# yaoyx689/RigGS

Hardware: AMD Instinct MI355X
Metric: train iters/sec (deform+raster fwd+bwd), 300k Gaussians @800x800 (higher is better)
Workload: dtype f32; 1 GPU; 300k Gaussians / 24-joint skeleton / 800x800, LBS-only, SH degree 3, anisotropic, one frame per GPU per step; num_gaussians=300000, num_joints=24, tile_instances_R=1963607, tile_lists=canonical: upstream's ceil(3 sigma) squares (the library default), parallelism=frames x1, launch=hipGraph replay

## Files before the change

### riggs_amd/csrc/pose_mlp.hip

```cpp
#include "fk_device.h"

namespace riggs {

#define PM_MAX_LAYERS 12
#define PM_MAX_W 256
#define PM_MAX_HEAD 320
#define PM_MAX_IN 320
#define PM_MAX_EMB 64
#define PM_RPW 8
#define PM_NG 16
#define PM_CPL 5

struct PoseMlpDesc {
  int depth;
  int width;
  int multires;
  int skip;
  int n_rot;
  const float* W[PM_MAX_LAYERS];
  const float* b[PM_MAX_LAYERS];
  const float *W_rot, *b_rot, *W_tr, *b_tr;
};

__device__ __forceinline__ int pm_in_dim(const PoseMlpDesc& d, int l, int emb) {
  if (l == 0) return emb;
  return (l - 1 == d.skip) ? d.width + emb : d.width;
}


__device__ __forceinline__ float pm_input(const PoseMlpDesc& d, const float* __restrict__ acts, int l, int emb, int i) {
  if (l == 0) return acts[i];
  if (l - 1 == d.skip) return (i < emb) ? acts[i] : acts[emb + (size_t)(l - 1) * d.width + (i - emb)];
  return acts[emb + (size_t)(l - 1) * d.width + i];
}

__global__ __launch_bounds__(64) void pm_embed_kernel(PoseMlpDesc d, const float* __restrict__ t, float* __restrict__ acts) {
  const int tid = threadIdx.x, emb = 1 + 2 * d.multires;
  if (tid < emb) {
    const float tv = t[0];
    float v = tv;
    if (tid > 0) {
      const int k = (tid - 1) >> 1;
      const float f = (float)(1 << k);
      v = ((tid - 1) & 1) ? cosf(tv * f) : sinf(tv * f);
    }
    acts[tid] = v;
  }
}

__global__ __launch_bounds__(256) void pm_layer_kernel(PoseMlpDesc d, int l, float* __restrict__ acts,
                                                       const float* __restrict__ rot_bias4,
                                                       float* __restrict__ rotation, float* __restrict__ translation) {
  const int lane = threadIdx.x & 63, wave = threadIdx.x >> 6;
  const int emb = 1 + 2 * d.multires;
  const bool heads = (l == d.depth);
  const int n_out = heads ? d.n_rot + 3 : d.width;
  const int r = blockIdx.x * 4 + wave;
  if (r >= n_out) return;
  const int in_dim = pm_in_dim(d, l, emb);
  const float* row;
  float bias;
  if (!heads) { row = d.W[l] + (size_t)r * in_dim; bias = d.b[l][r]; }
  else if (r < d.n_rot) { row = d.W_rot + (size_t)r * in_dim; bias = d.b_rot[r]; }
  else { row = d.W_tr + (size_t)(r - d.n_rot) * in_dim; bias = d.b_tr[r - d.n_rot]; }
  float acc = 0.f;
#pragma unroll
  for (int k = 0; k < PM_CPL; k++) {
    const int i = lane + 64 * k;
    if (i < in_dim) acc += row[i] * pm_input(d, acts, l, emb, i);
  }
  acc = wave_sum(acc);
  if (lane == 63) {
    const float v = acc + bias;
    if (!heads) acts[emb + (size_t)l * d.width + r] = fmaxf(v, 0.f);
    else if (r < d.n_rot) rotation[r] = rot_bias4 ? v + rot_bias4[r & 3] : v;
    else translation[r - d.n_rot] = v;
  }
}

#define PM_RG 8
__global__ __launch_bounds__(256) void pm_backward_step_kernel(PoseMlpDesc d, int l, const float* __restrict__ acts,
                                                               const float* __restrict__ g_rot,
                                                               const float* __restrict__ g_tr,
                                                               const float* __restrict__ dh_out ,
                                                               float* __restrict__ dh_in , float* __restrict__ dzs) {
  __shared__ float s_part[4][64];
  const int tid = threadIdx.x, lane = tid & 63, wave = tid >> 6;
  const int emb = 1 + 2 * d.multires;
  const bool heads = (l == d.depth);
  const int n_rows = heads ? d.n_rot + 3 : d.width;
  const int in_dim = pm_in_dim(d, l, emb);
  const int off = (l == d.skip) ? emb : 0;
  const int c = blockIdx.x * 64 + lane;
  const int rstep = 4 * PM_RG, r0 = blockIdx.y * 4 + wave;
  float acc = 0.f;
#pragma unroll 4
  for (int r = r0; r < n_rows; r += rstep) {
    float v;
    const float* row;
    if (heads) {
      v = (r < d.n_rot) ? g_rot[r] : g_tr[r - d.n_rot];
      row = (r < d.n_rot) ? d.W_rot + (size_t)r * in_dim : d.W_tr + (size_t)(r - d.n_rot) * in_dim;
    } else {
      const float h = acts[emb + (size_t)l * d.width + r];
      v = (h > 0.f) ? dh_out[off + r] : 0.f;
      row = d.W[l] + (size_t)r * in_dim;
      if (blockIdx.x == 0 && lane == 0) dzs[(size_t)l * d.width + r] = v;
    }
    if (l > 0 && c < in_dim) acc += row[c] * v;
  }
  if (l == 0) return;
  s_part[wave][lane] = acc;
  __syncthreads();
  if (wave == 0 && c < in_dim) atomicAdd(&dh_in[c], s_part[0][lane] + s_part[1][lane] + s_part[2][lane] + s_part[3][lane]);
}

struct PoseMlpGradDesc {
  int64_t w_off[PM_MAX_LAYERS + 2];
  int64_t b_off[PM_MAX_LAYERS + 2];
  int row_start[PM_MAX_LAYERS + 3];
};
__global__ __launch_bounds__(64) void pm_backward_weights_kernel(PoseMlpDesc d, PoseMlpGradDesc g,
                                                                 const float* __restrict__ acts,
                                                                 const float* __restrict__ dzs,
                                                                 const float* __restrict__ g_rot,
                                                                 const float* __restrict__ g_tr,
                                                                 float* __restrict__ flat) {
  const int emb = 1 + 2 * d.multires;
  const int nmat = d.depth + 2;
  int m = 0;
  while (m + 1 < nmat && (int)blockIdx.x >= g.row_start[m + 1]) m++;
  const int r = blockIdx.x - g.row_start[m];
  const int l = (m < d.depth) ? m : d.depth;
  const int in_dim = pm_in_dim(d, l, emb);
  const float v = (m < d.depth) ? dzs[(size_t)m * d.width + r] : (m == d.depth ? g_rot[r] : g_tr[r]);
  float* out = flat + g.w_off[m] + (size_t)r * in_dim;
  for (int c = threadIdx.x; c < in_dim; c += 64) out[c] = v * pm_input(d, acts, l, emb, c);
  if (threadIdx.x == 0) flat[g.b_off[m] + r] = v;
}


#define PMF_WAVES 8
#define PM_TRACE(i) do { if (trace && blockIdx.x == 0 && threadIdx.x == 0) trace[i] = wall_clock64(); } while (0)
#define PMF_SPIN_MAX (1u << 17)
typedef __attribute__((address_space(1))) unsigned long long pm_gu64;

__device__ __forceinline__ void pm_store_granule(unsigned long long* g, uint32_t tag, float value, bool local) {
  const unsigned long long x = ((unsigned long long)tag << 32) | (unsigned long long)__float_as_uint(value);
  if (local) asm volatile("global_store_dwordx2 %0, %1, off" ::"v"(g), "v"(x) : "memory");
  else __hip_atomic_store((pm_gu64*)g, x, __ATOMIC_RELAXED, __HIP_MEMORY_SCOPE_AGENT);
}

__device__ __forceinline__ void pm_sweep_issue(pm_gu64* g, int n, int lane, unsigned long long (&x)[4]) {
#pragma unroll
  for (int k = 0; k < 4; k++) {
    const int r = lane + 64 * k;
    x[k] = (r < n) ? __hip_atomic_load(g + r, __ATOMIC_RELAXED, __HIP_MEMORY_SCOPE_AGENT) : 0ull;
  }
}
__device__ __forceinline__ bool pm_sweep_check(const unsigned long long (&x)[4], int n, int lane, uint32_t tag,
                                               float (&v)[4]) {
  bool ok = true;
#pragma unroll
  for (int k = 0; k < 4; k++) {
    v[k] = __uint_as_float((uint32_t)x[k]);
    if (lane + 64 * k < n) ok &= ((uint32_t)(x[k] >> 32) == tag);
  }
  return __all(ok);
}
template <int NQ>
__device__ __forceinline__ bool pm_sweep_n(const unsigned long long* gran, int n, uint32_t tag, float (&v)[4],
                                           uint32_t* err, uint32_t* sticky, int lane) {
  pm_gu64* g = (pm_gu64*)gran;
  unsigned long long x[NQ][4];
#pragma unroll
  for (int q = 0; q < NQ; q++) {
    pm_sweep_issue(g, n, lane, x[q]);
    __builtin_amdgcn_s_sleep(2);
  }
  for (uint32_t spins = 0;; spins++) {
#pragma unroll
    for (int q = 0; q < NQ; q++) {
      if (pm_sweep_check(x[q], n, lane, tag, v)) return true;
      pm_sweep_issue(g, n, lane, x[q]);
    }
    if (spins > PMF_SPIN_MAX / NQ) {
      if (lane == 0) { atomicOr(err, 1u); if (sticky) atomicOr(sticky, 1u); }
      return false;
    }
  }
}
__device__ __forceinline__ bool pm_sweep(const unsigned long long* gran, int n, uint32_t tag, float (&v)[4],
                                         uint32_t* err, uint32_t* sticky, int lane, bool local = false) {
  return local ? pm_sweep_n<2>(gran, n, tag, v, err, sticky, lane) : pm_sweep_n<4>(gran, n, tag, v, err, sticky, lane);
}

#define PM_CHAIN_STRIDE 8
#define PM_MAX_CHAIN 64
__device__ __forceinline__ bool pm_chain_is_local(unsigned long long* xg, int rank, int n_chain, uint32_t tag, uint32_t* err,
                                                  uint32_t* sticky, int lane, int wave, int* s_word, int by = 0) {
  if (wave == by) {
    const uint32_t mine = __builtin_amdgcn_s_getreg(63508) & 0xFu;
    if (lane == 0) pm_store_granule(xg + rank, tag, __uint_as_float(mine), false);
    float v[4];
    const bool ok = pm_sweep(xg, n_chain, tag, v, err, sticky, lane);
    const bool same = ok && (lane >= n_chain || __float_as_uint(v[0]) == mine);
    const bool all_same = __all(same);
    if (lane == 0) *s_word = all_same ? 1 : 0;
  }
  __syncthreads();
  return *s_word != 0;
}

#define PM_FAULT_BIT 1u
__global__ __launch_bounds__(PMF_WAVES * 64) void pm_forward_fused_kernel(PoseMlpDesc d, const float* __restrict__ t,
                                                                          const float* __restrict__ rot_bias4,
                                                                          float* __restrict__ acts,
                                                                          unsigned long long* gran, uint32_t* gen,
                                                                          uint32_t* sticky, uint32_t* bwd_state, int bwd_words,
                                                                          float* __restrict__ rotation,
                                                                          float* __restrict__ translation,
                                                                          float* __restrict__ wt, int n_chain, int stride,
                                                                          unsigned long long* xcc_gran,
                                                                          unsigned long long* trace) {
  __shared__ float s_in[PM_MAX_IN];
  __shared__ int s_failed, s_local;
  const int lane = threadIdx.x & 63, wave = threadIdx.x >> 6;
  const int rank = (int)blockIdx.x / stride;
  if ((int)blockIdx.x % stride != 0 || rank >= n_chain) {
    __shared__ float s_t[32][33];
    const int emb_ = 1 + 2 * d.multires;
    const int tx = threadIdx.x & 31, ty = threadIdx.x >> 5;
    const int tiles_per = (PM_MAX_HEAD / 32) * (PM_MAX_W / 32);
    const int n_side = (int)gridDim.x - n_chain, side = (int)blockIdx.x - min(n_chain, (int)blockIdx.x / stride + 1);
    for (int tile = side; tile < d.depth * tiles_per; tile += n_side) {
      const int l = 1 + tile / tiles_per, tt = tile % tiles_per;
      const int r0 = (tt / (PM_MAX_W / 32)) * 32, c0 = (tt % (PM_MAX_W / 32)) * 32;
      const bool heads = (l == d.depth);
      const int in_dim = pm_in_dim(d, l, emb_);
      const int off = (l - 1 == d.skip) ? emb_ : 0;
      const int n_rows = heads ? d.n_rot + 3 : d.width;
#pragma unroll
      for (int h = 0; h < 2; h++) {
        const int r = r0 + ty + 16 * h, c = c0 + tx;
        float v = 0.f;
        if (r < n_rows && c < d.width) {
          const float* rp = !heads ? d.W[l] + (size_t)r * in_dim
                                   : (r < d.n_rot ? d.W_rot + (size_t)r * in_dim : d.W_tr + (size_t)(r - d.n_rot) * in_dim);
          v = rp[off + c];
        }
        s_t[ty + 16 * h][tx] = v;
      }
      __syncthreads();
#pragma unroll
      for (int h = 0; h < 2; h++)
        wt[((size_t)(l - 1) * PM_MAX_W + c0 + ty + 16 * h) * PM_MAX_HEAD + r0 + tx] = s_t[tx][ty + 16 * h];
      __syncthreads();
    }
    return;
  }
  const int row = rank * PMF_WAVES + wave;
  const int emb = 1 + 2 * d.multires;
  uint32_t* err = bwd_state;
  for (int i = rank * blockDim.x + threadIdx.x; i < bwd_words; i += n_chain * blockDim.x) bwd_state[i] = 0u;
  const uint32_t tag0 = __hip_atomic_load((__attribute__((address_space(1))) uint32_t*)gen, __ATOMIC_RELAXED,
                                          __HIP_MEMORY_SCOPE_AGENT) * 32u;
  float w[PM_MAX_LAYERS + 1][PM_CPL];
  float bias[PM_MAX_LAYERS + 1];
#pragma unroll
  for (int l = 0; l <= PM_MAX_LAYERS; l++) {
    bias[l] = 0.f;
#pragma unroll
    for (int k = 0; k < PM_CPL; k++) w[l][k] = 0.f;
    if (l <= d.depth) {
      const bool heads = (l == d.depth);
      const int n_out = heads ? d.n_rot + 3 : d.width;
      const int in_dim = pm_in_dim(d, l, emb);
      if (row < n_out) {
        const float* rp;
        if (!heads) { rp = d.W[l] + (size_t)row * in_dim; bias[l] = d.b[l][row]; }
        else if (row < d.n_rot) { rp = d.W_rot + (size_t)row * in_dim; bias[l] = d.b_rot[row]; }
        else { rp = d.W_tr + (size_t)(row - d.n_rot) * in_dim; bias[l] = d.b_tr[row - d.n_rot]; }
#pragma unroll
        for (int k = 0; k < PM_CPL; k++) {
          const int i = lane + 64 * k;
          if (i < in_dim) w[l][k] = rp[i];
        }
      }
    }
  }
  float embv = 0.f;
  if (lane < emb) {
    const float tv = t[0];
    embv = tv;
    if (lane > 0) {
      const int kf = (lane - 1) >> 1;
      const float f = (float)(1 << kf);
      embv = ((lane - 1) & 1) ? cosf(tv * f) : sinf(tv * f);
    }
    if (wave == 0) s_in[lane] = embv;
    if (wave == 0 && rank == 0) acts[lane] = embv;
  }
  if (threadIdx.x == 0) s_failed = 0;
  const bool fault = sticky != nullptr && rank == 1 && (sticky[1] & PM_FAULT_BIT) != 0u;
  PM_TRACE(0);
  const bool local = pm_chain_is_local(xcc_gran, rank, n_chain, tag0 + 31u, err, sticky, lane, wave, &s_local);
  const bool extra = rank * PMF_WAVES >= d.width;
#pragma unroll
  for (int l = 0; l <= PM_MAX_LAYERS; l++) {
    if (l <= d.depth && !(extra && l < d.depth)) {
      const bool heads = (l == d.depth);
      const int n_out = heads ? d.n_rot + 3 : d.width;
      const int in_dim = pm_in_dim(d, l, emb);
      PM_TRACE(1 + 2 * l);
      if (l > 0) {
        if (wave == 0) {
          float v[4];
          bool ok = (s_failed == 0);
          if (ok) ok = pm_sweep(gran + (size_t)(l - 1) * d.width, d.width, tag0 + (uint32_t)l, v, err, sticky, lane, local);
          if (!ok && lane == 0) s_failed = 1;
          const int off = (l - 1 == d.skip) ? emb : 0;
          if (off > 0 && lane < emb) s_in[lane] = embv;
#pragma unroll
          for (int k = 0; k < 4; k++) {
            const int r = lane + 64 * k;
            if (r < d.width) s_in[off + r] = v[k];
          }
        }
        __syncthreads();
      }
      float acc = 0.f;
#pragma unroll
      for (int k = 0; k < PM_CPL; k++) {
        const int i = lane + 64 * k;
        if (i < in_dim) acc += w[l][k] * s_in[i];
      }
      acc = wave_sum(acc);
      PM_TRACE(2 + 2 * l);
      if (lane == 63 && row < n_out) {
        float v = acc + bias[l];
        if (s_failed) v = __builtin_nanf("");
        if (!heads) {
          v = s_failed ? v : fmaxf(v, 0.f);
          if (!(fault && l == 1)) pm_store_granule(gran + (size_t)l * d.width + row, tag0 + (uint32_t)(l + 1), v, local);
          acts[emb + (size_t)l * d.width + row] = v;
        } else if (row < d.n_rot) {
          rotation[row] = rot_bias4 ? v + rot_bias4[row & 3] : v;
        } else {
          translation[row - d.n_rot] = v;
        }
      }
      __syncthreads();
    }
  }
  if (rank == 0 && threadIdx.x == 0)
    __hip_atomic_store((__attribute__((address_space(1))) uint32_t*)gen, tag0 / 32u + 1u, __ATOMIC_RELAXED,
                       __HIP_MEMORY_SCOPE_AGENT);
}

struct PmFkArgs {
  int J;
  const float *local_rot, *joints;
  const int32_t* parents;
  const float *dG, *g_nodes;
  const float* transforms;
  float *dq_out, *dgt_out;
  const float* fixed_coef;
  float* fixed_loss_out;
};

__global__ __launch_bounds__(256) void pm_fixed_add_kernel(int J, const float* __restrict__ local_rot, const float* __restrict__ coef,
                                                           float* __restrict__ dq, float* __restrict__ loss_out) {
  __shared__ float s_p[4];
  float ss = 0.f;
  for (int t = threadIdx.x; t < 4 * J; t += 256) {
    const float d = local_rot[t] - ((t & 3) == 0 ? 1.f : 0.f);
    if (coef) dq[t] += coef[0] * d;
    ss += d * d;
  }
  for (int o = 32; o > 0; o >>= 1) ss += __shfl_xor(ss, o);
  if ((threadIdx.x & 63) == 0) s_p[threadIdx.x >> 6] = ss;
  __syncthreads();
  if (threadIdx.x == 0 && loss_out) loss_out[0] = ((s_p[0] + s_p[1]) + (s_p[2] + s_p[3])) / (float)(4 * J);
}
__global__ __launch_bounds__(256) void pm_add_kernel(int n, const float* __restrict__ src, float* __restrict__ dst) {
  const int i = blockIdx.x * 256 + threadIdx.x;
  if (i < n) dst[i] += src[i];
}

#undef PM_FAULT_BIT
#define PM_FAULT_BIT 2u
__global__ __launch_bounds__(PMF_WAVES * 64) void pm_backward_fused_kernel(PoseMlpDesc d, PoseMlpGradDesc g, PmFkArgs fk,
                                                                           const float* __restrict__ acts,
                                                                           const float* __restrict__ g_rot,
                                                                           const float* __restrict__ g_tr,
                                                                           unsigned long long* gran, uint32_t* err,
                                                                           uint32_t* sticky, uint32_t* gen, float* __restrict__ flat,
                                                                           const float* __restrict__ wt, int n_chain, int stride,
                                                                           unsigned long long* xcc_gran,
                                                                           unsigned long long* trace) {
  __shared__ float s_v[PM_MAX_HEAD];
  __shared__ int s_failed, s_local;
  const int lane = threadIdx.x & 63, wave = threadIdx.x >> 6;
  const int rank = (int)blockIdx.x / stride;
  if ((int)blockIdx.x % stride != 0 || rank >= n_chain) return;
  const int col = rank * PMF_WAVES + wave;
  const bool extra = rank * PMF_WAVES >= d.width;
  const int emb = 1 + 2 * d.multires;
  const int n_head = d.n_rot + 3;
  const uint32_t tag0 = __hip_atomic_load((__attribute__((address_space(1))) uint32_t*)gen, __ATOMIC_RELAXED,
                                          __HIP_MEMORY_SCOPE_AGENT) * 32u;
  __shared__ float s_gq[4 * MAX_J + 4];
  FkIn fin;
  if (fk.J > 0 && wave == 0) fk_load(fk.J, fk.local_rot, fk.joints, fk.parents, fk.dG, fk.g_nodes, fin, fk.transforms);
  float wc[PM_MAX_LAYERS + 1][4];
  float wc_head = 0.f;
#pragma unroll
  for (int l = 1; l <= PM_MAX_LAYERS; l++) {
#pragma unroll
    for (int k = 0; k < 4; k++) wc[l][k] = 0.f;
    if (l <= d.depth && col < d.width) {
      const int n_rows = (l == d.depth) ? n_head : d.width;
      const float* rp = wt + ((size_t)(l - 1) * PM_MAX_W + col) * PM_MAX_HEAD;
#pragma unroll
      for (int k = 0; k < 4; k++) {
        const int r = lane + 64 * k;
        if (r < n_rows) wc[l][k] = rp[r];
      }
      if (l == d.depth && lane + 256 < n_rows) wc_head = rp[lane + 256];
    }
  }
  __shared__ float s_acts[PM_MAX_EMB + PM_MAX_LAYERS * PM_MAX_W];
  __shared__ float s_late[PM_MAX_LAYERS + 1];
  for (int i = threadIdx.x; i < emb + d.depth * d.width; i += blockDim.x) s_acts[i] = acts[i];
  if (threadIdx.x == 0) s_failed = 0;
  const bool fault = sticky != nullptr && rank == 1 && (sticky[1] & PM_FAULT_BIT) != 0u;
  PM_TRACE(0);
  if (fk.J > 0 && wave == 0) {
    FkLane f;
    fk_wave_forward(fk.J, fin, f, fk.transforms != nullptr);
    float dq[4];
    fk_wave_backward(fk.J, fin, f, dq);
    if (lane < fk.J) {
#pragma unroll
      for (int e = 0; e < 4; e++) s_gq[4 * lane + e] = dq[e];
    }
  }
  const bool local = pm_chain_is_local(xcc_gran, rank, n_chain, tag0 + 31u, err, sticky, lane, wave, &s_local, 1);
  if (fk.J > 0) {
    if (threadIdx.x < 3) {
      float sgt = g_tr ? g_tr[threadIdx.x] : 0.f;
      if (fk.g_nodes) for (int k = 0; k < fk.J; k++) sgt += fk.g_nodes[3 * k + threadIdx.x];
      s_gq[4 * fk.J + threadIdx.x] = sgt;
      if (rank == 0 && fk.dgt_out) fk.dgt_out[threadIdx.x] = sgt;
    }
    __syncthreads();
    if (g_rot && (int)threadIdx.x < 4 * fk.J) s_gq[threadIdx.x] += g_rot[threadIdx.x];
    if ((fk.fixed_coef || fk.fixed_loss_out) && wave == 0) {
      float ss = 0.f;
      for (int i = lane; i < 4 * fk.J; i += 64) {
        const float dqf = fk.local_rot[i] - ((i & 3) == 0 ? 1.f : 0.f);
        ss += dqf * dqf;
      }
      for (int o = 32; o > 0; o >>= 1) ss += __shfl_xor(ss, o);
      if (rank == 0 && lane == 0 && fk.fixed_loss_out) fk.fixed_loss_out[0] = ss / (float)(4 * fk.J);
    }
    if (fk.fixed_coef && (int)threadIdx.x < 4 * fk.J)
      s_gq[threadIdx.x] += fk.fixed_coef[0] * (fk.local_rot[threadIdx.x] - ((threadIdx.x & 3) == 0 ? 1.f : 0.f));
    __syncthreads();
    if (rank == 0 && fk.dq_out && (int)threadIdx.x < 4 * fk.J) fk.dq_out[threadIdx.x] = s_gq[threadIdx.x];
  }
  PM_TRACE(1);
#pragma unroll
  for (int l = PM_MAX_LAYERS; l >= 0; l--) {
    if (l <= d.depth && !(extra && l < d.depth)) {
      const bool heads = (l == d.depth);
      const int n_rows = heads ? n_head : d.width;
      const int in_dim = pm_in_dim(d, l, emb);
      PM_TRACE(2 + 2 * (d.depth - l));
      if (wave == 0) {
        if (heads) {
#pragma unroll
          for (int k = 0; k < PM_MAX_HEAD / 64; k++) {
            const int r = lane + 64 * k;
            if (fk.J > 0) s_v[r] = (r < n_head) ? s_gq[r] : 0.f;
            else s_v[r] = (r < d.n_rot) ? g_rot[r] : (r < n_head ? g_tr[r - d.n_rot] : 0.f);
          }
        } else {
          float h[4];
#pragma unroll
          for (int k = 0; k < 4; k++) {
            const int r = lane + 64 * k;
            h[k] = (r < d.width) ? s_acts[emb + (size_t)l * d.width + r] : 0.f;
          }
          float v[4];
          bool ok = (s_failed == 0);
          if (ok) ok = pm_sweep(gran + (size_t)l * d.width, d.width, tag0 + (uint32_t)(l + 1), v, err, sticky, lane, local);
          if (!ok && lane == 0) s_failed = 1;
#pragma unroll
          for (int k = 0; k < 4; k++) {
            const int r = lane + 64 * k;
            if (r < PM_MAX_W) s_v[r] = (r < d.width && h[k] > 0.f) ? v[k] : 0.f;
          }
        }
      }
      __syncthreads();
      PM_TRACE(3 + 2 * (d.depth - l));
      float sv[4];
#pragma unroll
      for (int k = 0; k < 4; k++) sv[k] = s_v[lane + 64 * k];
      const float sv_head = heads ? s_v[lane + 256] : 0.f;
      float vr = (col < n_rows) ? s_v[col] : 0.f;
      if (s_failed) vr = __builtin_nanf("");
      __syncthreads();
      if (l >= 1) {
        float acc = 0.f;
#pragma unroll
        for (int k = 0; k < 4; k++) {
          const int r = lane + 64 * k;
          if (r < n_rows) acc += wc[l][k] * sv[k];
        }
        if (heads && lane + 256 < n_rows) acc += wc_head * sv_head;
        acc = wave_sum(acc);
        if (lane == 63 && col < d.width && !(fault && l == 2)) pm_store_granule(gran + (size_t)(l - 1) * d.width + col, tag0 + (uint32_t)l, acc, local);
      }
      if (wave == 0) {
        if (lane == 0) s_late[l] = vr;
      } else if (col < n_rows) {
        int m = l, r = col;
        if (heads && col >= d.n_rot) { m = d.depth + 1; r = col - d.n_rot; }
        float* out = flat + g.w_off[m] + (size_t)r * in_dim;
        for (int c = lane; c < in_dim; c += 64) out[c] = vr * pm_input(d, s_acts, l, emb, c);
        if (lane == 0) flat[g.b_off[m] + r] = vr;
      }
    }
  }
  PM_TRACE(4 + 2 * d.depth);
  __syncthreads();
  {
    const int col0 = rank * PMF_WAVES;
#pragma unroll
    for (int l = PM_MAX_LAYERS; l >= 0; l--) {
      if (l <= d.depth && (l % PMF_WAVES) == wave) {
        const bool heads = (l == d.depth);
        const int n_rows = heads ? n_head : d.width;
        const int in_dim = pm_in_dim(d, l, emb);
        if (col0 < n_rows) {
          int m = l, r = col0;
          if (heads && col0 >= d.n_rot) { m = d.depth + 1; r = col0 - d.n_rot; }
          const float vr = s_late[l];
          float* out = flat + g.w_off[m] + (size_t)r * in_dim;
          for (int c = lane; c < in_dim; c += 64) out[c] = vr * pm_input(d, s_acts, l, emb, c);
          if (lane == 0) flat[g.b_off[m] + r] = vr;
        }
      }
    }
  }
  if (wave == 0) {
    PM_TRACE(5 + 2 * d.depth);
    if (rank == 0 && lane == 0)
      __hip_atomic_store((__attribute__((address_space(1))) uint32_t*)gen, tag0 / 32u + 1u, __ATOMIC_RELAXED,
                         __HIP_MEMORY_SCOPE_AGENT);
  }
}

}

using namespace riggs;

extern "C" {

static int pm_fill(PoseMlpDesc& d, int32_t depth, int32_t width, int32_t multires, int32_t skip, int32_t n_rot,
                   const float* const* weights, const float* const* biases, const float* W_rot, const float* b_rot,
                   const float* W_tr, const float* b_tr) {
  RIGGS_REQUIRE(depth >= 1 && depth <= PM_MAX_LAYERS, "PoseMLP depth out of range");
  RIGGS_REQUIRE(width >= 1 && width <= PM_MAX_W, "PoseMLP width must be <= 256");
  RIGGS_REQUIRE(multires >= 0 && 1 + 2 * multires <= PM_MAX_EMB, "PoseMLP multires out of range");
  RIGGS_REQUIRE(n_rot >= 1 && n_rot <= 4 * MAX_J_WIDE, "PoseMLP rotation head too wide");
  d.depth = depth; d.width = width; d.multires = multires; d.skip = skip; d.n_rot = n_rot;
  for (int l = 0; l < depth; l++) { d.W[l] = weights[l]; d.b[l] = biases[l]; }
  d.W_rot = W_rot; d.b_rot = b_rot; d.W_tr = W_tr; d.b_tr = b_tr;
  return 0;
}

static int g_pm_one_xcd = 1;
static int pm_chain_stride(const void* kernel, int n_chain) {
  int per_cu = 0, dev = 0, cus = 0;
  if (hipOccupancyMaxActiveBlocksPerMultiprocessor(&per_cu, kernel, PMF_WAVES * 64, 0) != hipSuccess || hipGetDevice(&dev) != hipSuccess ||
      hipDeviceGetAttribute(&cus, hipDeviceAttributeMultiprocessorCount, dev) != hipSuccess) {
    (void)hipGetLastError();
    return 1;
  }
  return (per_cu * (cus / PM_CHAIN_STRIDE) >= n_chain) ? PM_CHAIN_STRIDE : 1;
}

int riggs_pose_mlp_set_placement(int32_t one_xcd) { g_pm_one_xcd = one_xcd ? 1 : 0; return 0; }

static unsigned long long* g_pm_trace = nullptr;
int riggs_pose_mlp_set_trace(void* dev_u64x128) { g_pm_trace = (unsigned long long*)dev_u64x128; return 0; }

static bool pm_one_launch(int32_t width, int32_t n_rot) {
  if (option(OPT_POSE_MLP_LAYERED)) return false;
  if (n_rot > 4 * MAX_J) return false;
  return n_rot + 3 <= width || (width >= 128 && n_rot + 3 <= PM_MAX_HEAD);
}
static size_t pm_acts_core(int32_t depth, int32_t width, int32_t multires) {
  return ((size_t)(1 + 2 * multires) + (size_t)depth * width + 63) & ~(size_t)63;
}
static size_t pm_xcc_offset(int32_t depth, int32_t width) { return (2 * (size_t)depth * width + 4 + 63) & ~(size_t)63; }
static size_t pm_sync_floats(int32_t depth, int32_t width) {
  return pm_xcc_offset(depth, width) + 2 * PM_MAX_CHAIN;
}
size_t riggs_pose_mlp_sync_bytes(int32_t depth, int32_t width) { return pm_sync_floats(depth, width) * sizeof(float); }
size_t riggs_pose_mlp_status_word(int32_t depth, int32_t width) { return 2 * (size_t)depth * width + 1; }
size_t riggs_pose_mlp_acts_floats(int32_t depth, int32_t width, int32_t multires) {
  return pm_acts_core(depth, width, multires) + 2 * pm_sync_floats(depth, width) + (size_t)depth * PM_MAX_W * PM_MAX_HEAD;
}

int riggs_pose_mlp_forward(int32_t depth, int32_t width, int32_t multires, int32_t skip, int32_t n_rot,
                           const float* const* weights, const float* const* biases, const float* W_rot,
                           const float* b_rot, const float* W_tr, const float* b_tr, const float* t,
                           const float* rot_bias4, void* sync_state, float* acts, float* rotation,
                           float* translation, riggs_stream stream) {
  PoseMlpDesc d;
  int rc = pm_fill(d, depth, width, multires, skip, n_rot, weights, biases, W_rot, b_rot, W_tr, b_tr);
  if (rc) return rc;
  hipStream_t s = (hipStream_t)stream;
  ProfScope ps(PROF_POSE_FWD, s);
  if (pm_one_launch(width, n_rot)) {
    const size_t sf = pm_sync_floats(depth, width);
    float* own = acts + pm_acts_core(depth, width, multires);
    float* fs = (float*)sync_state;
    if (fs == nullptr) {
      fs = own;
      RIGGS_HIP_CHECK(hipMemsetAsync(fs, 0, sf * sizeof(float), s));
    }
    const int n_chain = ((width > n_rot + 3 ? width : n_rot + 3) + PMF_WAVES - 1) / PMF_WAVES;
    static int stride_f[PM_MAX_CHAIN + 1];
    if (stride_f[n_chain] == 0) stride_f[n_chain] = pm_chain_stride(reinterpret_cast<const void*>(pm_forward_fused_kernel), n_chain);
    const int stride = g_pm_one_xcd ? stride_f[n_chain] : 1;
    hipLaunchKernelGGL(pm_forward_fused_kernel, dim3(stride > 1 ? n_chain * stride : n_chain + 64), dim3(PMF_WAVES * 64), 0, s, d, t, rot_bias4, acts,
                       (unsigned long long*)fs, (uint32_t*)(fs + 2 * (size_t)depth * width),
                       sync_state ? (uint32_t*)(fs + 2 * (size_t)depth * width) + 1 : nullptr, (uint32_t*)(own + sf), (int)sf,
                       rotation, translation, own + 2 * sf, n_chain, stride, (unsigned long long*)(fs + pm_xcc_offset(depth, width)),
                       g_pm_trace);
    RIGGS_HIP_CHECK(hipGetLastError());
    return 0;
  }
  hipLaunchKernelGGL(pm_embed_kernel, dim3(1), dim3(64), 0, s, d, t, acts);
  for (int l = 0; l <= depth; l++) {
    const int n_out = (l == depth) ? n_rot + 3 : width;
    hipLaunchKernelGGL(pm_layer_kernel, dim3((n_out + 3) / 4), dim3(256), 0, s, d, l, acts, rot_bias4, rotation, translation);
  }
  RIGGS_HIP_CHECK(hipGetLastError());
  return 0;
}

static size_t pm_bwd_core(int32_t depth, int32_t width) {
  return ((size_t)depth * width + (size_t)(depth + 1) * PM_MAX_IN + 1) & ~(size_t)1;
}
size_t riggs_pose_mlp_backward_workspace_floats(int32_t depth, int32_t width, int32_t multires) {
  (void)multires;
  return pm_bwd_core(depth, width);
}

static int pm_backward_impl(int32_t depth, int32_t width, int32_t multires, int32_t skip, int32_t n_rot,
                            const float* const* weights, const float* const* biases, const float* W_rot,
                            const float* b_rot, const float* W_tr, const float* b_tr, float* acts,
                            const float* g_rotation, const float* g_translation, float* workspace,
                            float* flat_grads, void* sync_state, riggs_stream stream, PmFkArgs fk) {
  PoseMlpDesc d;
  int rc = pm_fill(d, depth, width, multires, skip, n_rot, weights, biases, W_rot, b_rot, W_tr, b_tr);
  if (rc) return rc;
  hipStream_t s = (hipStream_t)stream;
  const int emb = 1 + 2 * multires;
  float* dzs = workspace;
  float* dh = workspace + (size_t)depth * width;
  PoseMlpGradDesc g;
  int64_t o = 0;
  int rows = 0;
  for (int l = 0; l < depth; l++) {
    const int in_l = (l == 0) ? emb : ((l - 1 == skip) ? width + emb : width);
    g.w_off[l] = o; o += (int64_t)width * in_l;
    g.b_off[l] = o; o += width;
    g.row_start[l] = rows; rows += width;
  }
  const int in_h = (depth - 1 == skip) ? width + emb : width;
  g.w_off[depth] = o; o += (int64_t)n_rot * in_h;
  g.b_off[depth] = o; o += n_rot;
  g.row_start[depth] = rows; rows += n_rot;
  g.w_off[depth + 1] = o; o += (int64_t)3 * in_h;
  g.b_off[depth + 1] = o; o += 3;
  g.row_start[depth + 1] = rows; rows += 3;
  g.row_start[depth + 2] = rows;
  ProfScope ps(PROF_POSE_BWD, s);
  if (pm_one_launch(width, n_rot)) {
    float* tail = acts + pm_acts_core(depth, width, multires) + pm_sync_floats(depth, width);
    const int nr = width > n_rot + 3 ? width : n_rot + 3;
    const int n_chain = (nr + PMF_WAVES - 1) / PMF_WAVES;
    static int stride_b[PM_MAX_CHAIN + 1];
    if (stride_b[n_chain] == 0) stride_b[n_chain] = pm_chain_stride(reinterpret_cast<const void*>(pm_backward_fused_kernel), n_chain);
    const int stride = g_pm_one_xcd ? stride_b[n_chain] : 1;
    hipLaunchKernelGGL(pm_backward_fused_kernel, dim3(n_chain * stride), dim3(PMF_WAVES * 64), 0, s, d, g, fk,
                       acts, g_rotation, g_translation, (unsigned long long*)(tail + 4), (uint32_t*)tail,
                       sync_state ? (uint32_t*)sync_state + 2 * (size_t)depth * width + 1 : nullptr,
                       (uint32_t*)tail + 1, flat_grads, tail + pm_sync_floats(depth, width), n_chain, stride,
                       (unsigned long long*)(tail + pm_xcc_offset(depth, width)), g_pm_trace ? g_pm_trace + 64 : nullptr);
    RIGGS_HIP_CHECK(hipGetLastError());
    return 0;
  }
  if (fk.J > 0) {
    RIGGS_REQUIRE(fk.dq_out && fk.dgt_out, "riggs_pose_mlp_backward_fk needs dL_dlocal_rot and dL_dglobal_trans");
    if (g_translation) RIGGS_HIP_CHECK(hipMemcpyAsync(fk.dgt_out, g_translation, 12, hipMemcpyDeviceToDevice, s));
    else RIGGS_HIP_CHECK(hipMemsetAsync(fk.dgt_out, 0, 12, s));
    int rc2 = riggs_fk_backward(fk.J, fk.local_rot, fk.joints, fk.parents, fk.dG, fk.g_nodes, fk.dq_out, fk.dgt_out, stream);
    if (rc2) return rc2;
    if (g_rotation) {
      hipLaunchKernelGGL(pm_add_kernel, dim3((4 * fk.J + 255) / 256), dim3(256), 0, s, 4 * fk.J, g_rotation, fk.dq_out);
      RIGGS_HIP_CHECK(hipGetLastError());
    }
    if (fk.fixed_coef || fk.fixed_loss_out) {
      hipLaunchKernelGGL(pm_fixed_add_kernel, dim3(1), dim3(256), 0, s, fk.J, fk.local_rot, fk.fixed_coef, fk.dq_out, fk.fixed_loss_out);
      RIGGS_HIP_CHECK(hipGetLastError());
    }
    g_rotation = fk.dq_out; g_translation = fk.dgt_out;
  }
  RIGGS_HIP_CHECK(hipMemsetAsync(dh, 0, (size_t)(depth + 1) * PM_MAX_IN * sizeof(float), s));
  for (int l = depth; l >= 0; l--) {
    const int in_l = (l == 0) ? emb : ((l - 1 == skip) ? width + emb : width);
    const float* dh_out = (l == depth) ? nullptr : dh + (size_t)(l + 1) * PM_MAX_IN;
    hipLaunchKernelGGL(pm_backward_step_kernel, dim3(l == 0 ? 1 : (in_l + 63) / 64, PM_RG), dim3(256), 0, s, d, l, acts,
                       g_rotation, g_translation, dh_out, dh + (size_t)l * PM_MAX_IN, dzs);
  }
  hipLaunchKernelGGL(pm_backward_weights_kernel, dim3(rows), dim3(64), 0, s, d, g, acts, dzs, g_rotation,
                     g_translation, flat_grads);
  RIGGS_HIP_CHECK(hipGetLastError());
  return 0;
}

int riggs_pose_mlp_backward(int32_t depth, int32_t width, int32_t multires, int32_t skip, int32_t n_rot,
                            const float* const* weights, const float* const* biases, const float* W_rot,
                            const float* b_rot, const float* W_tr, const float* b_tr, float* acts,
                            const float* g_rotation, const float* g_translation, float* workspace,
                            float* flat_grads, void* sync_state, riggs_stream stream) {
  PmFkArgs fk;
  memset(&fk, 0, sizeof(fk));
  return pm_backward_impl(depth, width, multires, skip, n_rot, weights, biases, W_rot, b_rot, W_tr, b_tr, acts, g_rotation,
                          g_translation, workspace, flat_grads, sync_state, stream, fk);
}

int riggs_pose_mlp_backward_fk(int32_t depth, int32_t width, int32_t multires, int32_t skip, int32_t n_rot,
                               const float* const* weights, const float* const* biases, const float* W_rot,
                               const float* b_rot, const float* W_tr, const float* b_tr, float* acts, int32_t num_joints,
                               const float* local_rot, const float* joints, const int32_t* parents, const float* transforms,
                               const float* dL_dtransforms, const float* dL_dd_nodes, const float* g_rotation,
                               const float* g_translation, float* dL_dlocal_rot, float* dL_dglobal_trans,
                               const float* template_fixed_coef, float* template_fixed_loss, float* workspace,
                               float* flat_grads, void* sync_state, riggs_stream stream) {
  RIGGS_REQUIRE(num_joints >= 1 && num_joints <= MAX_J_WIDE && 4 * num_joints == n_rot, "the rotation head must predict one quaternion per joint");
  RIGGS_REQUIRE(local_rot && joints && parents && dL_dtransforms, "riggs_pose_mlp_backward_fk: missing chain input");
  PmFkArgs fk;
  fk.J = num_joints; fk.local_rot = local_rot; fk.joints = joints; fk.parents = parents; fk.dG = dL_dtransforms;
  fk.g_nodes = dL_dd_nodes; fk.dq_out = dL_dlocal_rot; fk.dgt_out = dL_dglobal_trans; fk.transforms = transforms;
  fk.fixed_coef = template_fixed_coef; fk.fixed_loss_out = template_fixed_loss;
  return pm_backward_impl(depth, width, multires, skip, n_rot, weights, biases, W_rot, b_rot, W_tr, b_tr, acts, g_rotation,
                          g_translation, workspace, flat_grads, sync_state, stream, fk);
}

}
```

Before: 3094 iters/s.

## Trim barriers and hoist loads in fused pose-MLP forward/backward chain kernels

Replaces __syncthreads with a bare lgkmcnt wait plus s_barrier, and issues the generation, fault and input loads early so their latency overlaps other setup. The XCC-locality publish moves to a separate wave ahead of the weight loads, and the check becomes an inline spin. In backward, the FK translation-gradient sum and the regularisation loss move to wave 2, the late weight-gradient writes are folded into the main layer loop, and one barrier phase for layer 0 is dropped. The aim is to shorten the serial latency of the tiny chained MLP kernels, at the cost of subtle memory-ordering risk from the weaker barriers.

```diff
diff --git a/riggs_amd/csrc/pose_mlp.hip b/riggs_amd/csrc/pose_mlp.hip
--- a/riggs_amd/csrc/pose_mlp.hip
+++ b/riggs_amd/csrc/pose_mlp.hip
@@ -197,18 +197,43 @@
 
 #define PM_CHAIN_STRIDE 8
 #define PM_MAX_CHAIN 64
-__device__ __forceinline__ bool pm_chain_is_local(unsigned long long* xg, int rank, int n_chain, uint32_t tag, uint32_t* err,
-                                                  uint32_t* sticky, int lane, int wave, int* s_word, int by = 0) {
+#define PM_LDS_BARRIER() asm volatile("s_waitcnt lgkmcnt(0)\n\ts_barrier" ::: "memory")
+__device__ __forceinline__ void pm_need(uint32_t& v) { asm volatile("" : "+v"(v)); }
+__device__ __forceinline__ void pm_need(float& v) { asm volatile("" : "+v"(v)); }
+__device__ __forceinline__ uint32_t pm_xcc_id() { return __builtin_amdgcn_s_getreg(63508) & 0xFu; }
+__device__ __forceinline__ void pm_chain_publish(unsigned long long* xg, int rank, uint32_t tag, int lane) {
+  if (lane == 0) pm_store_granule(xg + rank, tag, __uint_as_float(pm_xcc_id()), false);
+}
+__device__ __forceinline__ bool pm_chain_is_local(unsigned long long* xg, int n_chain, uint32_t tag, uint32_t* err,
+                                                  uint32_t* sticky, int lane, int wave, int* s_word, int by) {
   if (wave == by) {
-    const uint32_t mine = __builtin_amdgcn_s_getreg(63508) & 0xFu;
-    if (lane == 0) pm_store_granule(xg + rank, tag, __uint_as_float(mine), false);
-    float v[4];
-    const bool ok = pm_sweep(xg, n_chain, tag, v, err, sticky, lane);
-    const bool same = ok && (lane >= n_chain || __float_as_uint(v[0]) == mine);
-    const bool all_same = __all(same);
+    pm_gu64* g = (pm_gu64*)xg + min(lane, n_chain - 1);
+    unsigned long long x[4];
+#pragma unroll
+    for (int q = 0; q < 4; q++) {
+      x[q] = __hip_atomic_load(g, __ATOMIC_RELAXED, __HIP_MEMORY_SCOPE_AGENT);
+      __builtin_amdgcn_s_sleep(2);
+    }
+    bool all_same = false;
+    for (uint32_t spins = 0;; spins++) {
+      bool ok = false;
+#pragma unroll
+      for (int q = 0; q < 4; q++) {
+        if (!ok && __all((uint32_t)(x[q] >> 32) == tag)) {
+          ok = true;
+          all_same = __all((uint32_t)x[q] == pm_xcc_id());
+        }
+        if (!ok) x[q] = __hip_atomic_load(g, __ATOMIC_RELAXED, __HIP_MEMORY_SCOPE_AGENT);
+      }
+      if (ok) break;
+      if (spins > PMF_SPIN_MAX / 4) {
+        if (lane == 0) { atomicOr(err, 1u); if (sticky) atomicOr(sticky, 1u); }
+        break;
+      }
+    }
     if (lane == 0) *s_word = all_same ? 1 : 0;
   }
-  __syncthreads();
+  PM_LDS_BARRIER();
   return *s_word != 0;
 }
 
@@ -262,9 +287,15 @@
   const int row = rank * PMF_WAVES + wave;
   const int emb = 1 + 2 * d.multires;
   uint32_t* err = bwd_state;
+  float tv = t[0];
+  uint32_t genw = __hip_atomic_load((__attribute__((address_space(1))) uint32_t*)gen, __ATOMIC_RELAXED, __HIP_MEMORY_SCOPE_AGENT);
+  uint32_t hookw = 0u;
+  if (sticky != nullptr && rank == 1) hookw = sticky[1];
   for (int i = rank * blockDim.x + threadIdx.x; i < bwd_words; i += n_chain * blockDim.x) bwd_state[i] = 0u;
-  const uint32_t tag0 = __hip_atomic_load((__attribute__((address_space(1))) uint32_t*)gen, __ATOMIC_RELAXED,
-                                          __HIP_MEMORY_SCOPE_AGENT) * 32u;
+  pm_need(tv); pm_need(genw); pm_need(hookw);
+  const uint32_t tag0 = genw * 32u;
+  const bool fault = (hookw & PM_FAULT_BIT) != 0u;
+  if (wave == 1) pm_chain_publish(xcc_gran, rank, tag0 + 31u, lane);
   float w[PM_MAX_LAYERS + 1][PM_CPL];
   float bias[PM_MAX_LAYERS + 1];
 #pragma unroll
@@ -290,21 +321,19 @@
     }
   }
   float embv = 0.f;
-  if (lane < emb) {
-    const float tv = t[0];
+  if (wave == 0 && lane < emb) {
     embv = tv;
     if (lane > 0) {
       const int kf = (lane - 1) >> 1;
       const float f = (float)(1 << kf);
       embv = ((lane - 1) & 1) ? cosf(tv * f) : sinf(tv * f);
     }
-    if (wave == 0) s_in[lane] = embv;
-    if (wave == 0 && rank == 0) acts[lane] = embv;
+    s_in[lane] = embv;
+    if (rank == 0) acts[lane] = embv;
   }
   if (threadIdx.x == 0) s_failed = 0;
-  const bool fault = sticky != nullptr && rank == 1 && (sticky[1] & PM_FAULT_BIT) != 0u;
   PM_TRACE(0);
-  const bool local = pm_chain_is_local(xcc_gran, rank, n_chain, tag0 + 31u, err, sticky, lane, wave, &s_local);
+  const bool local = pm_chain_is_local(xcc_gran, n_chain, tag0 + 31u, err, sticky, lane, wave, &s_local, 1);
   const bool extra = rank * PMF_WAVES >= d.width;
 #pragma unroll
   for (int l = 0; l <= PM_MAX_LAYERS; l++) {
@@ -327,7 +356,7 @@
             if (r < d.width) s_in[off + r] = v[k];
           }
         }
-        __syncthreads();
+        PM_LDS_BARRIER();
       }
       float acc = 0.f;
 #pragma unroll
@@ -350,7 +379,7 @@
           translation[row - d.n_rot] = v;
         }
       }
-      __syncthreads();
+      PM_LDS_BARRIER();
     }
   }
   if (rank == 0 && threadIdx.x == 0)
@@ -408,11 +437,29 @@
   const bool extra = rank * PMF_WAVES >= d.width;
   const int emb = 1 + 2 * d.multires;
   const int n_head = d.n_rot + 3;
-  const uint32_t tag0 = __hip_atomic_load((__attribute__((address_space(1))) uint32_t*)gen, __ATOMIC_RELAXED,
-                                          __HIP_MEMORY_SCOPE_AGENT) * 32u;
+  uint32_t genw = __hip_atomic_load((__attribute__((address_space(1))) uint32_t*)gen, __ATOMIC_RELAXED, __HIP_MEMORY_SCOPE_AGENT);
+  uint32_t hookw = 0u;
+  if (sticky != nullptr && rank == 1) hookw = sticky[1];
+  float pre_grot = 0.f, pre_coef = 0.f, pre_lr = 0.f;
+  if (fk.J > 0 && (int)threadIdx.x < 4 * fk.J) {
+    if (g_rot) pre_grot = g_rot[threadIdx.x];
+    if (fk.fixed_coef) { pre_coef = fk.fixed_coef[0]; pre_lr = fk.local_rot[threadIdx.x]; }
+  }
   __shared__ float s_gq[4 * MAX_J + 4];
   FkIn fin;
-  if (fk.J > 0 && wave == 0) fk_load(fk.J, fk.local_rot, fk.joints, fk.parents, fk.dG, fk.g_nodes, fin, fk.transforms);
+  if (fk.J > 0 && wave == 0) {
+    fk_load(fk.J, fk.local_rot, fk.joints, fk.parents, fk.dG, fk.g_nodes, fin, fk.transforms);
+#pragma unroll
+    for (int e = 0; e < 12; e++) { pm_need(fin.dG[e]); pm_need(fin.G[e]); }
+#pragma unroll
+    for (int e = 0; e < 3; e++) { pm_need(fin.c[e]); pm_need(fin.x[e]); pm_need(fin.gn[e]); }
+#pragma unroll
+    for (int e = 0; e < 4; e++) pm_need(fin.q[e]);
+  }
+  if (wave == 1) {
+    pm_need(genw);
+    pm_chain_publish(xcc_gran, rank, genw * 32u + 31u, lane);
+  }
   float wc[PM_MAX_LAYERS + 1][4];
   float wc_head = 0.f;
 #pragma unroll
@@ -431,10 +478,12 @@
     }
   }
   __shared__ float s_acts[PM_MAX_EMB + PM_MAX_LAYERS * PM_MAX_W];
-  __shared__ float s_late[PM_MAX_LAYERS + 1];
-  for (int i = threadIdx.x; i < emb + d.depth * d.width; i += blockDim.x) s_acts[i] = acts[i];
+  {
+    const int first = (fk.J > 0) ? 64 : 0;
+    if ((int)threadIdx.x >= first)
+      for (int i = (int)threadIdx.x - first; i < emb + d.depth * d.width; i += (int)blockDim.x - first) s_acts[i] = acts[i];
+  }
   if (threadIdx.x == 0) s_failed = 0;
-  const bool fault = sticky != nullptr && rank == 1 && (sticky[1] & PM_FAULT_BIT) != 0u;
   PM_TRACE(0);
   if (fk.J > 0 && wave == 0) {
     FkLane f;
@@ -446,31 +495,58 @@
       for (int e = 0; e < 4; e++) s_gq[4 * lane + e] = dq[e];
     }
   }
-  const bool local = pm_chain_is_local(xcc_gran, rank, n_chain, tag0 + 31u, err, sticky, lane, wave, &s_local, 1);
+  if (fk.J > 0 && wave == 2) {
+    const bool want_loss = rank == 0 && fk.fixed_loss_out != nullptr;
+    float gx[3] = {0.f, 0.f, 0.f}, lr[4] = {0.f, 0.f, 0.f, 0.f};
+    if (fk.g_nodes) {
+#pragma unroll
+      for (int k = 0; k < 3; k++) gx[k] = fk.g_nodes[min(lane + 64 * k, 3 * fk.J - 1)];
+    }
+    if (want_loss) {
+#pragma unroll
+      for (int k = 0; k < 4; k++) lr[k] = fk.local_rot[min(lane + 64 * k, 4 * fk.J - 1)];
+    }
+    if (fk.g_nodes) {
+#pragma unroll
+      for (int k = 0; k < 3; k++)
+        if (lane + 64 * k < 3 * fk.J) s_v[lane + 64 * k] = gx[k];
+      __builtin_amdgcn_wave_barrier();
+    }
+    if (lane < 3) {
+      float sgt = g_tr ? g_tr[lane] : 0.f;
+      if (fk.g_nodes) for (int k = 0; k < fk.J; k++) sgt += s_v[3 * k + lane];
+      s_gq[4 * fk.J + lane] = sgt;
+      if (rank == 0 && fk.dgt_out) fk.dgt_out[lane] = sgt;
+    }
+    if (want_loss) {
+      float ss = 0.f;
+#pragma unroll
+      for (int k = 0; k < 4; k++) {
+        const int i = lane + 64 * k;
+        if (i < 4 * fk.J) {
+          const float dqf = lr[k] - ((i & 3) == 0 ? 1.f : 0.f);
+          ss += dqf * dqf;
+        }
+      }
+      for (int o = 32; o > 0; o >>= 1) ss += __shfl_xor(ss, o);
+      if (lane == 0) fk.fixed_loss_out[0] = ss / (float)(4 * fk.J);
+    }
+  }
+  pm_need(genw); pm_need(hookw);
+  const uint32_t tag0 = genw * 32u;
+  const bool fault = (hookw & PM_FAULT_BIT) != 0u;
+  const bool local = pm_chain_is_local(xcc_gran, n_chain, tag0 + 31u, err, sticky, lane, wave, &s_local, 1);
   if (fk.J > 0) {
-    if (threadIdx.x < 3) {
-      float sgt = g_tr ? g_tr[threadIdx.x] : 0.f;
-      if (fk.g_nodes) for (int k = 0; k < fk.J; k++) sgt += fk.g_nodes[3 * k + threadIdx.x];
-      s_gq[4 * fk.J + threadIdx.x] = sgt;
-      if (rank == 0 && fk.dgt_out) fk.dgt_out[threadIdx.x] = sgt;
-    }
-    __syncthreads();
-    if (g_rot && (int)threadIdx.x < 4 * fk.J) s_gq[threadIdx.x] += g_rot[threadIdx.x];
-    if ((fk.fixed_coef || fk.fixed_loss_out) && wave == 0) {
-      float ss = 0.f;
-      for (int i = lane; i < 4 * fk.J; i += 64) {
-        const float dqf = fk.local_rot[i] - ((i & 3) == 0 ? 1.f : 0.f);
-        ss += dqf * dqf;
-      }
-      for (int o = 32; o > 0; o >>= 1) ss += __shfl_xor(ss, o);
-      if (rank == 0 && lane == 0 && fk.fixed_loss_out) fk.fixed_loss_out[0] = ss / (float)(4 * fk.J);
-    }
-    if (fk.fixed_coef && (int)threadIdx.x < 4 * fk.J)
-      s_gq[threadIdx.x] += fk.fixed_coef[0] * (fk.local_rot[threadIdx.x] - ((threadIdx.x & 3) == 0 ? 1.f : 0.f));
-    __syncthreads();
+    if ((int)threadIdx.x < 4 * fk.J) {
+      if (g_rot) s_gq[threadIdx.x] += pre_grot;
+      if (fk.fixed_coef) s_gq[threadIdx.x] += pre_coef * (pre_lr - ((threadIdx.x & 3) == 0 ? 1.f : 0.f));
+    }
+    PM_LDS_BARRIER();
     if (rank == 0 && fk.dq_out && (int)threadIdx.x < 4 * fk.J) fk.dq_out[threadIdx.x] = s_gq[threadIdx.x];
   }
   PM_TRACE(1);
+  const int col0 = rank * PMF_WAVES;
+  float acc_prev = 0.f;
 #pragma unroll
   for (int l = PM_MAX_LAYERS; l >= 0; l--) {
     if (l <= d.depth && !(extra && l < d.depth)) {
@@ -478,42 +554,48 @@
       const int n_rows = heads ? n_head : d.width;
       const int in_dim = pm_in_dim(d, l, emb);
       PM_TRACE(2 + 2 * (d.depth - l));
-      if (wave == 0) {
-        if (heads) {
-#pragma unroll
-          for (int k = 0; k < PM_MAX_HEAD / 64; k++) {
-            const int r = lane + 64 * k;
-            if (fk.J > 0) s_v[r] = (r < n_head) ? s_gq[r] : 0.f;
-            else s_v[r] = (r < d.n_rot) ? g_rot[r] : (r < n_head ? g_tr[r - d.n_rot] : 0.f);
-          }
-        } else {
-          float h[4];
-#pragma unroll
-          for (int k = 0; k < 4; k++) {
-            const int r = lane + 64 * k;
-            h[k] = (r < d.width) ? s_acts[emb + (size_t)l * d.width + r] : 0.f;
-          }
-          float v[4];
-          bool ok = (s_failed == 0);
-          if (ok) ok = pm_sweep(gran + (size_t)l * d.width, d.width, tag0 + (uint32_t)(l + 1), v, err, sticky, lane, local);
-          if (!ok && lane == 0) s_failed = 1;
-#pragma unroll
-          for (int k = 0; k < 4; k++) {
-            const int r = lane + 64 * k;
-            if (r < PM_MAX_W) s_v[r] = (r < d.width && h[k] > 0.f) ? v[k] : 0.f;
+      float vr, vr0 = 0.f;
+      if (l == 0) {
+        PM_TRACE(3 + 2 * d.depth);
+        vr = (col < d.width && s_acts[emb + col] > 0.f) ? acc_prev : 0.f;
+        if (s_failed) vr = __builtin_nanf("");
+      } else {
+        if (wave == 0) {
+          if (heads) {
+#pragma unroll
+            for (int k = 0; k < PM_MAX_HEAD / 64; k++) {
+              const int r = lane + 64 * k;
+              if (fk.J > 0) s_v[r] = (r < n_head) ? s_gq[r] : 0.f;
+              else s_v[r] = (r < d.n_rot) ? g_rot[r] : (r < n_head ? g_tr[r - d.n_rot] : 0.f);
+            }
+          } else {
+            float h[4];
+#pragma unroll
+            for (int k = 0; k < 4; k++) {
+              const int r = lane + 64 * k;
+              h[k] = (r < d.width) ? s_acts[emb + (size_t)l * d.width + r] : 0.f;
+            }
+            float v[4];
+            bool ok = (s_failed == 0);
+            if (ok) ok = pm_sweep(gran + (size_t)l * d.width, d.width, tag0 + (uint32_t)(l + 1), v, err, sticky, lane, local);
+            if (!ok && lane == 0) s_failed = 1;
+#pragma unroll
+            for (int k = 0; k < 4; k++) {
+              const int r = lane + 64 * k;
+              if (r < PM_MAX_W) s_v[r] = (r < d.width && h[k] > 0.f) ? v[k] : 0.f;
+            }
           }
         }
-      }
-      __syncthreads();
-      PM_TRACE(3 + 2 * (d.depth - l));
-      float sv[4];
-#pragma unroll
-      for (int k = 0; k < 4; k++) sv[k] = s_v[lane + 64 * k];
-      const float sv_head = heads ? s_v[lane + 256] : 0.f;
-      float vr = (col < n_rows) ? s_v[col] : 0.f;
-      if (s_failed) vr = __builtin_nanf("");
-      __syncthreads();
-      if (l >= 1) {
+        PM_LDS_BARRIER();
+        PM_TRACE(3 + 2 * (d.depth - l));
+        float sv[4];
+#pragma unroll
+        for (int k = 0; k < 4; k++) sv[k] = s_v[lane + 64 * k];
+        const float sv_head = heads ? s_v[lane + 256] : 0.f;
+        vr = (col < n_rows) ? s_v[col] : 0.f;
+        vr0 = (col0 < n_rows) ? s_v[col0] : 0.f;
+        if (s_failed) vr = vr0 = __builtin_nanf("");
+        PM_LDS_BARRIER();
         float acc = 0.f;
 #pragma unroll
         for (int k = 0; k < 4; k++) {
@@ -522,40 +604,26 @@
         }
         if (heads && lane + 256 < n_rows) acc += wc_head * sv_head;
         acc = wave_sum(acc);
-        if (lane == 63 && col < d.width && !(fault && l == 2)) pm_store_granule(gran + (size_t)(l - 1) * d.width + col, tag0 + (uint32_t)l, acc, local);
-      }
-      if (wave == 0) {
-        if (lane == 0) s_late[l] = vr;
-      } else if (col < n_rows) {
-        int m = l, r = col;
-        if (heads && col >= d.n_rot) { m = d.depth + 1; r = col - d.n_rot; }
-        float* out = flat + g.w_off[m] + (size_t)r * in_dim;
-        for (int c = lane; c < in_dim; c += 64) out[c] = vr * pm_input(d, s_acts, l, emb, c);
-        if (lane == 0) flat[g.b_off[m] + r] = vr;
+        if (l >= 2 && lane == 63 && col < d.width && !(fault && l == 2)) pm_store_granule(gran + (size_t)(l - 1) * d.width + col, tag0 + (uint32_t)l, acc, local);
+        acc_prev = __builtin_bit_cast(float, __builtin_amdgcn_readlane(__builtin_bit_cast(int, acc), 63));
+      }
+      const int other = (l == 0) ? -1 : 1 + l % (PMF_WAVES - 1);
+#pragma unroll 1
+      for (int pass = 0; pass < 2; pass++) {
+        if (pass == 0 ? (wave == 0 && l != 0) : (wave != other)) continue;
+        const int c_row = pass == 0 ? col : col0;
+        const float v = pass == 0 ? vr : vr0;
+        if (c_row < n_rows) {
+          int m = l, r = c_row;
+          if (heads && c_row >= d.n_rot) { m = d.depth + 1; r = c_row - d.n_rot; }
+          float* out = flat + g.w_off[m] + (size_t)r * in_dim;
+          for (int c = lane; c < in_dim; c += 64) out[c] = v * pm_input(d, s_acts, l, emb, c);
+          if (lane == 0) flat[g.b_off[m] + r] = v;
+        }
       }
     }
   }
   PM_TRACE(4 + 2 * d.depth);
-  __syncthreads();
-  {
-    const int col0 = rank * PMF_WAVES;
-#pragma unroll
-    for (int l = PM_MAX_LAYERS; l >= 0; l--) {
-      if (l <= d.depth && (l % PMF_WAVES) == wave) {
-        const bool heads = (l == d.depth);
-        const int n_rows = heads ? n_head : d.width;
-        const int in_dim = pm_in_dim(d, l, emb);
-        if (col0 < n_rows) {
-          int m = l, r = col0;
-          if (heads && col0 >= d.n_rot) { m = d.depth + 1; r = col0 - d.n_rot; }
-          const float vr = s_late[l];
-          float* out = flat + g.w_off[m] + (size_t)r * in_dim;
-          for (int c = lane; c < in_dim; c += 64) out[c] = vr * pm_input(d, s_acts, l, emb, c);
-          if (lane == 0) flat[g.b_off[m] + r] = vr;
-        }
-      }
-    }
-  }
   if (wave == 0) {
     PM_TRACE(5 + 2 * d.depth);
     if (rank == 0 && lane == 0)
```

Result: no change. 3099 iters/s (median of 3 runs) (+0.2%).
